# uber-research/deep-neuroevolution

Measured on NVIDIA H100. Metric: env-steps/sec across ES population (whole box), higher is better.
Workload: dtype f32

## Files before the change

### deep-neuroevolution_b200/csrc/gemv_bulk.cu

```cuda
#include <climits>
#include "common.cuh"
#include "forward.cuh"
#include "epilogue.cuh"
#include "wgmma.cuh"

using namespace wg;

int g_dne_gemv_bulk = 1;
int g_dne_gemv_ctas_per_sm = 2;
int g_dne_gemv_grid = 0;
int g_dne_gemv_stages = 5;

constexpr int GB_CONSUMERS = 256;
constexpr int GB_THREADS = GB_CONSUMERS + 32;
constexpr int GB_STAGES = 8;
constexpr int GB_STAGE_BYTES = 16384;
constexpr int GB_RPR = 4;
constexpr int GU_BLK = DNE_GEMV_BLOCK_ROWS;
constexpr int GU_VEC = 8;
constexpr int GU_VB = 4;
constexpr int GU_MIN_N = 64;
constexpr int GU_XS_LD_MAX = GU_BLK + 4096 / GU_MIN_N;
constexpr int GU_XS_FLOATS = GU_VEC * GU_XS_LD_MAX > (1024 / GU_MIN_N) * GU_VB * (GU_MIN_N + 4)
                                 ? GU_VEC * GU_XS_LD_MAX : (1024 / GU_MIN_N) * GU_VB * (GU_MIN_N + 4);
constexpr int GU_PLAN_BYTES_PER_GROUP = 8 + 5 * 4;

__device__ __forceinline__ int gu_cover(const int* pb0, const int* pb1, int n_groups, int b, int first, int cap, int* out,
                                        int lane) {
    int total = 0;
    for (int h0 = 0; h0 < n_groups; h0 += 32) {
        const int h = h0 + lane;
        const bool c = h < n_groups && pb0[h] <= b && b <= pb1[h];
        const unsigned m = __ballot_sync(0xffffffffu, c);
        const int ord = total + __popc(m & ((1u << lane) - 1u));
        if (c && ord >= first && ord < first + cap) out[ord - first] = h;
        total += __popc(m);
    }
    __syncwarp();
    return total;
}

template <int G>
__global__ void __launch_bounds__(GB_THREADS, 2)
gemv_union_kernel(SlotArgs sa, GemvSrc src, const float* __restrict__ X, int64_t x_slot_stride, int K, int N,
                  int n_pieces, int n_groups, int n_slots, float* __restrict__ part, int n_stages,
                  const float* __restrict__ tpart, int t_split) {
    constexpr int CAP = GU_VEC / G;
    extern __shared__ uint8_t smem_raw[];
    uint8_t* smem = (uint8_t*)(((uintptr_t)smem_raw + 127) & ~(uintptr_t)127);
    float* stage_base = reinterpret_cast<float*>(smem);
    int64_t* pE0 = reinterpret_cast<int64_t*>(smem + n_stages * GB_STAGE_BYTES);
    int* pb0 = reinterpret_cast<int*>(pE0 + n_groups);
    int* pb1 = pb0 + n_groups;
    int* psort = pb1 + n_groups;
    int* pstart = psort + n_groups;
    int* ppre = pstart + n_groups;
    __shared__ uint64_t full_bar[GB_STAGES], empty_bar[GB_STAGES];
    __shared__ __align__(16) float xs[GU_XS_FLOATS];
    __shared__ int cov_c[CAP], cov_p[CAP];
    __shared__ int rho_c[CAP];
    __shared__ int s_total, s_row0, s_nelem, s_items;

    const int tid = threadIdx.x, warp = tid >> 5, lane = tid & 31;
    const int NQ = N >> 2;
    const int RW = GB_CONSUMERS / NQ;
    const int RB = GB_RPR * RW;
    const int XS_LD = GU_BLK + RB;
    pdl_trigger();

    if (tid == 0) {
        for (int s = 0; s < n_stages; ++s) {
            mbar_init(&full_bar[s], 1);
            mbar_init(&empty_bar[s], GB_CONSUMERS / 32);
        }
        fence_mbar_init();
    }
    for (int g = tid; g < n_groups; g += GB_THREADS) {
        const int slot0 = g * G;
        bool any = false;
#pragma unroll
        for (int m = 0; m < G; ++m) any = any || (slot0 + m < n_slots && slot_active(sa, slot0 + m));
        const int64_t E0 = (src.idx64 ? src.idx64[slot0] : (src.idx32 ? (int64_t)src.idx32[slot0] * src.mul : 0)) + src.off;
        pE0[g] = E0;
        pb0[g] = any ? (int)(E0 / N / GU_BLK) : INT_MAX;
        pb1[g] = any ? (int)((E0 + (int64_t)K * N - 1) / N / GU_BLK) : -1;
    }
    __syncthreads();
    for (int g = tid; g < n_groups; g += GB_THREADS) {
        const int key = pb0[g];
        int r = 0;
        for (int h = 0; h < n_groups; ++h) {
            const int kh = pb0[h];
            r += (kh < key) || (kh == key && h < g);
        }
        psort[r] = g;
    }
    __syncthreads();
    if (warp == 0) {
        int carry_max = -1, carry_sum = 0;
        for (int i0 = 0; i0 < n_groups; i0 += 32) {
            const int i = i0 + lane;
            const int g = i < n_groups ? psort[i] : 0;
            const int b0 = i < n_groups ? pb0[g] : INT_MAX, b1 = i < n_groups ? pb1[g] : -1;
            int mx = b1;
#pragma unroll
            for (int d = 1; d < 32; d <<= 1) {
                const int o = __shfl_up_sync(0xffffffffu, mx, d);
                if (lane >= d) mx = max(mx, o);
            }
            int before = __shfl_up_sync(0xffffffffu, mx, 1);
            if (lane == 0) before = -1;
            before = max(before, carry_max);
            const int start = max(b0, before + 1);
            const int add = (b0 != INT_MAX && b1 >= start) ? b1 - start + 1 : 0;
            int sum = add;
#pragma unroll
            for (int d = 1; d < 32; d <<= 1) {
                const int o = __shfl_up_sync(0xffffffffu, sum, d);
                if (lane >= d) sum += o;
            }
            if (i < n_groups) { pstart[i] = start; ppre[i] = carry_sum + sum - add; }
            carry_sum += __shfl_sync(0xffffffffu, sum, 31);
            carry_max = max(carry_max, __shfl_sync(0xffffffffu, mx, 31));
        }
        if (lane == 0) s_items = carry_sum;
    }
    __syncthreads();
    const int n_items = s_items;
    auto item_block = [&](int q) {
        int lo = 0, hi = n_groups;
        while (lo < hi) {
            const int mid = (lo + hi) >> 1;
            if (ppre[mid] <= q) lo = mid + 1; else hi = mid;
        }
        return pstart[lo - 1] + (q - ppre[lo - 1]);
    };
    auto pass_range = [&](int b, const int* gl, int ng, int64_t& row0, int& n_elem) {
        int64_t r_first = INT64_MAX, e_last = 0;
        for (int i = 0; i < ng; ++i) {
            const int64_t E0 = pE0[gl[i]];
            r_first = min(r_first, E0 / N);
            e_last = max(e_last, (E0 + (int64_t)K * N + 3) & ~(int64_t)3);
        }
        const int64_t blk0 = (int64_t)b * GU_BLK;
        row0 = max(r_first, blk0);
        const int64_t e_end = min(e_last, (blk0 + GU_BLK) * N);
        n_elem = (int)(e_end - row0 * N);
    };

    if (warp == GB_CONSUMERS / 32) {
        uint32_t it = 0;
        for (int item = blockIdx.x; item < n_items; item += gridDim.x) {
            const int b = item_block(item);
            int total = CAP;
            for (int first = 0; first < total; first += CAP) {
                total = gu_cover(pb0, pb1, n_groups, b, first, CAP, cov_p, lane);
                int64_t row0;
                int n_elem;
                pass_range(b, cov_p, min(CAP, total - first), row0, n_elem);
                const float* gsrc = src.base + row0 * N;
                for (int e0 = 0; e0 < n_elem; e0 += RB * N, ++it) {
                    if (lane == 0) {
                        const int s = it % n_stages;
                        mbar_wait(&empty_bar[s], ((it / n_stages) & 1) ^ 1);
                        const uint32_t bytes = (uint32_t)min(RB * N, n_elem - e0) * 4;
                        mbar_arrive_expect_tx(&full_bar[s], bytes);
                        bulk_g2s(stage_base + (size_t)s * (GB_STAGE_BYTES / 4), gsrc + e0, bytes, &full_bar[s]);
                    }
                }
                __syncwarp();
            }
        }
        return;
    }

    pdl_wait();
    const int t = tid % NQ, rw = tid / NQ;
    const int red_ld = N + 4;
    float* red = xs;
    uint32_t it = 0;
    for (int item = blockIdx.x; item < n_items; item += gridDim.x) {
        const int b = item_block(item);
        int total = CAP;
        for (int first = 0; first < total; first += CAP) {
            if (warp == 0) {
                const int tot = gu_cover(pb0, pb1, n_groups, b, first, CAP, cov_c, lane);
                if (lane == 0) {
                    const int ng = min(CAP, tot - first);
                    int64_t row0;
                    int n_elem;
                    pass_range(b, cov_c, ng, row0, n_elem);
                    s_total = tot;
                    s_row0 = (int)(row0 - (int64_t)b * GU_BLK);
                    s_nelem = n_elem;
                    for (int i = 0; i < ng; ++i) rho_c[i] = (int)(pE0[cov_c[i]] % N);
                }
            }
            named_bar_sync(1, GB_CONSUMERS);
            total = s_total;
            const int ng = min(CAP, total - first), nv = ng * G;
            const int lrow0 = s_row0, n_elem = s_nelem;
            for (int i = tid; i < nv * XS_LD; i += GB_CONSUMERS) {
                const int v = i / XS_LD, L = i - v * XS_LD - 1;
                const int g = cov_c[v / G], slot = g * G + v % G;
                const int64_t k = (int64_t)b * GU_BLK + L - pE0[g] / N;
                xs[v * XS_LD + L + 1] = (k >= 0 && k < K && slot < n_slots) ? X[(int64_t)slot * x_slot_stride + k] : 0.0f;
            }
            named_bar_sync(1, GB_CONSUMERS);

            float acc[GU_VEC][4];
#pragma unroll
            for (int v = 0; v < GU_VEC; ++v)
#pragma unroll
                for (int c = 0; c < 4; ++c) acc[v][c] = 0.0f;

            for (int e0 = 0; e0 < n_elem; e0 += RB * N, ++it) {
                const int s = it % n_stages;
                const int stage_elems = min(RB * N, n_elem - e0);
                const int rl0 = rw * GB_RPR;
                const int xb0 = lrow0 + e0 / N + rl0;
                mbar_wait(&full_bar[s], (it / n_stages) & 1);
                const uint32_t rows_a = wg::smem_u32(stage_base) + s * GB_STAGE_BYTES + (rl0 * NQ + t) * 16;
                float4 w[GB_RPR];
#pragma unroll
                for (int j = 0; j < GB_RPR; ++j)
                    w[j] = ((rl0 + j) * N + 4 * t < stage_elems) ? wg::lds128(rows_a + j * NQ * 16) : make_float4(0.f, 0.f, 0.f, 0.f);
#pragma unroll
                for (int gi = 0; gi < CAP; ++gi) {
                    if (gi < ng) {
                        const int rho = rho_c[gi];
                        const bool p0 = 4 * t < rho, p1 = 4 * t + 1 < rho, p2 = 4 * t + 2 < rho, p3 = 4 * t + 3 < rho;
#pragma unroll
                        for (int m = 0; m < G; ++m) {
                            const int v = gi * G + m;
                            float xm[GB_RPR + 1];
#pragma unroll
                            for (int j = 0; j <= GB_RPR; ++j) xm[j] = xs[v * XS_LD + xb0 + j];
#pragma unroll
                            for (int j = 0; j < GB_RPR; ++j) {
                                acc[v][0] = fmaf(p0 ? xm[j] : xm[j + 1], w[j].x, acc[v][0]);
                                acc[v][1] = fmaf(p1 ? xm[j] : xm[j + 1], w[j].y, acc[v][1]);
                                acc[v][2] = fmaf(p2 ? xm[j] : xm[j + 1], w[j].z, acc[v][2]);
                                acc[v][3] = fmaf(p3 ? xm[j] : xm[j + 1], w[j].w, acc[v][3]);
                            }
                        }
                    }
                }
                __syncwarp();
                if (lane == 0) mbar_arrive(&empty_bar[s]);
            }
            for (int vb0 = 0; vb0 < nv; vb0 += GU_VB) {
                named_bar_sync(1, GB_CONSUMERS);
#pragma unroll
                for (int v = 0; v < GU_VEC; ++v) {
                    if (v >= vb0 && v < vb0 + GU_VB && v < nv) {
                        const int rho = rho_c[v / G];
                        float* row = red + (rw * GU_VB + (v - vb0)) * red_ld;
#pragma unroll
                        for (int c = 0; c < 4; ++c) {
                            const int n = 4 * t + c - rho;
                            row[n < 0 ? n + N : n] = acc[v][c];
                        }
                    }
                }
                named_bar_sync(1, GB_CONSUMERS);
                for (int i = tid; i < GU_VB * N; i += GB_CONSUMERS) {
                    const int vl = i / N, n = i - vl * N, v = vb0 + vl;
                    if (v >= nv) break;
                    const int g = cov_c[v / G], m = v % G, slot = g * G + m;
                    const int piece = b - pb0[g];
                    float sum = 0.0f;
                    for (int w2 = 0; w2 < RW; ++w2) sum += red[(w2 * GU_VB + vl) * red_ld + n];
                    if (tpart) {
                        float ts = 0.0f;
                        if (slot < n_slots)
                            for (int j = piece; j < t_split; j += n_pieces) ts += tpart[((int64_t)j * n_slots + slot) * N + n];
                        sum = fmaf(slot < n_slots ? sa.scale[slot] : 0.0f, sum, ts);
                    }
                    part[(((int64_t)g * n_pieces + piece) * G + m) * N + n] = sum;
                }
            }
            for (int gi = 0; gi < ng; ++gi) {
                const int g = cov_c[gi];
                if (pb1[g] != b) continue;
                for (int piece = b - pb0[g] + 1; piece < n_pieces; ++piece)
                    for (int i = tid; i < G * N; i += GB_CONSUMERS) {
                        const int m = i / N, n = i - m * N, slot = g * G + m;
                        float ts = 0.0f;
                        if (tpart && slot < n_slots)
                            for (int j = piece; j < t_split; j += n_pieces) ts += tpart[((int64_t)j * n_slots + slot) * N + n];
                        part[(((int64_t)g * n_pieces + piece) * G + m) * N + n] = ts;
                    }
            }
            named_bar_sync(1, GB_CONSUMERS);
        }
    }
}

int dne_gemv_pieces(int K) { return (K + 1 + GU_BLK - 1) / GU_BLK + 1; }

int dne_launch_gemv_union(const SlotArgs& sa, const GemvSrc& src, int G, const float* X, int64_t x_slot_stride, int K,
                          int N, int n_pieces, int n_slots, float* part, int sm_count, cudaStream_t st,
                          const float* fold_theta, int fold_n_split) {
    if (N % 4 != 0 || N < GU_MIN_N || N * 4 > GB_STAGE_BYTES || (GB_CONSUMERS % (N / 4)) != 0) return DNE_ERR_UNSUP;
    const int RW = GB_CONSUMERS / (N / 4);
    if (GB_RPR * RW * N * 4 != GB_STAGE_BYTES || n_pieces != dne_gemv_pieces(K) || (G != 1 && G != 2)) return DNE_ERR_UNSUP;
    const int n_groups = (n_slots + G - 1) / G;
    if (n_groups <= 0) return 0;
    const size_t static_smem = (size_t)GU_XS_FLOATS * 4 + 1024;
    const size_t plan = (size_t)n_groups * GU_PLAN_BYTES_PER_GROUP + 128;
    const size_t per_sm = 227 * 1024;
    int cps = g_dne_gemv_ctas_per_sm, n_stages = 0;
    for (; cps >= 1; --cps) {
        const size_t budget = per_sm / cps - 1024;
        n_stages = budget > static_smem + plan ? (int)((budget - static_smem - plan) / GB_STAGE_BYTES) : 0;
        if (n_stages > g_dne_gemv_stages) n_stages = g_dne_gemv_stages;
        if (n_stages >= 2) break;
    }
    if (cps < 1) return DNE_ERR_UNSUP;
    const size_t smem = (size_t)n_stages * GB_STAGE_BYTES + plan;
    int grid = cps * sm_count;
    if (g_dne_gemv_grid > 0 && grid > g_dne_gemv_grid) grid = g_dne_gemv_grid;
    int dev = 0;
    cudaGetDevice(&dev);
    static bool attr_done_dev[64][3] = {};
    bool* attr_done = attr_done_dev[dev < 64 ? dev : 63];
    auto launch = [&](auto kern) -> int {
        if (!attr_done[G]) {
            cudaFuncSetAttribute(kern, cudaFuncAttributePreferredSharedMemoryCarveout, cudaSharedmemCarveoutMaxShared);
            if (cudaFuncSetAttribute(kern, cudaFuncAttributeMaxDynamicSharedMemorySize, (int)(per_sm - static_smem - 1024)) != cudaSuccess)
                return DNE_ERR_CUDA;
            attr_done[G] = true;
        }
        if (dne_launch_chain(kern, dim3(grid), dim3(GB_THREADS), smem, st, true, sa, src, X, x_slot_stride, K, N, n_pieces,
                             n_groups, n_slots, part, n_stages, fold_theta, fold_theta ? fold_n_split : 0) != cudaSuccess)
            return DNE_ERR_CUDA;
        return 0;
    };
    return G == 2 ? launch(gemv_union_kernel<2>) : launch(gemv_union_kernel<1>);
}
```

Baseline: 345,300.

## Move x-vector staging to producer warp with double-buffered cp.async and mbarriers

The producer warp now computes pass metadata and loads the x-vector slices into a double-buffered shared buffer with cp.async zero-fill, signalling consumers through new mbarriers. This takes the cover computation, the x gather and two named barriers off the consumer critical path and lets the next pass's x load overlap the current pass's compute. It halves GU_VB so the reduction scratch fits inside one x buffer, which adds an extra reduction round for larger vector counts. Static shared memory grows because the x buffer is now doubled, which may cut the number of weight stages that fit.

```diff
diff --git a/deep-neuroevolution_b200/csrc/gemv_bulk.cu b/deep-neuroevolution_b200/csrc/gemv_bulk.cu
--- a/deep-neuroevolution_b200/csrc/gemv_bulk.cu
+++ b/deep-neuroevolution_b200/csrc/gemv_bulk.cu
@@ -18,12 +18,24 @@
 constexpr int GB_RPR = 4;
 constexpr int GU_BLK = DNE_GEMV_BLOCK_ROWS;
 constexpr int GU_VEC = 8;
-constexpr int GU_VB = 4;
+constexpr int GU_VB = 2;
 constexpr int GU_MIN_N = 64;
 constexpr int GU_XS_LD_MAX = GU_BLK + 4096 / GU_MIN_N;
-constexpr int GU_XS_FLOATS = GU_VEC * GU_XS_LD_MAX > (1024 / GU_MIN_N) * GU_VB * (GU_MIN_N + 4)
-                                 ? GU_VEC * GU_XS_LD_MAX : (1024 / GU_MIN_N) * GU_VB * (GU_MIN_N + 4);
+constexpr int GU_XS_BUF = GU_VEC * GU_XS_LD_MAX;
+static_assert((1024 / GU_MIN_N) * GU_VB * (GU_MIN_N + 4) <= GU_XS_BUF, "the reduction of every N fits an x buffer");
 constexpr int GU_PLAN_BYTES_PER_GROUP = 8 + 5 * 4;
+
+struct GuPass {
+    int b, total, ng, row0, n_elem;
+    int cov[GU_VEC], rho[GU_VEC];
+};
+
+__device__ __forceinline__ void cp_async4_zfill(float* dst, const float* src, bool ok) {
+    asm volatile("cp.async.ca.shared.global [%0], [%1], 4, %2;" ::"r"(smem_u32(dst)), "l"(src), "r"(ok ? 4 : 0) : "memory");
+}
+__device__ __forceinline__ void cp_async_mbar_arrive_noinc(uint64_t* bar) {
+    asm volatile("cp.async.mbarrier.arrive.noinc.shared::cta.b64 [%0];" ::"r"(smem_u32(bar)) : "memory");
+}
 
 __device__ __forceinline__ int gu_cover(const int* pb0, const int* pb1, int n_groups, int b, int first, int cap, int* out,
                                         int lane) {
@@ -38,6 +50,12 @@
     }
     __syncwarp();
     return total;
+}
+
+__device__ __forceinline__ void gu_pass_extent(int b, int64_t r_first, int64_t e_last, int N, int64_t& row0, int& n_elem) {
+    const int64_t blk0 = (int64_t)b * GU_BLK;
+    row0 = max(r_first, blk0);
+    n_elem = (int)(min(e_last, (blk0 + GU_BLK) * N) - row0 * N);
 }
 
 template <int G>
@@ -55,11 +73,11 @@
     int* psort = pb1 + n_groups;
     int* pstart = psort + n_groups;
     int* ppre = pstart + n_groups;
-    __shared__ uint64_t full_bar[GB_STAGES], empty_bar[GB_STAGES];
-    __shared__ __align__(16) float xs[GU_XS_FLOATS];
-    __shared__ int cov_c[CAP], cov_p[CAP];
-    __shared__ int rho_c[CAP];
-    __shared__ int s_total, s_row0, s_nelem, s_items;
+    __shared__ uint64_t full_bar[GB_STAGES], empty_bar[GB_STAGES], xs_full[2], xs_empty[2];
+    __shared__ __align__(16) float xs[2][GU_XS_BUF];
+    __shared__ GuPass pass[2];
+    __shared__ int cov_p[CAP];
+    __shared__ int s_items;
 
     const int tid = threadIdx.x, warp = tid >> 5, lane = tid & 31;
     const int NQ = N >> 2;
@@ -72,6 +90,10 @@
         for (int s = 0; s < n_stages; ++s) {
             mbar_init(&full_bar[s], 1);
             mbar_init(&empty_bar[s], GB_CONSUMERS / 32);
+        }
+        for (int s = 0; s < 2; ++s) {
+            mbar_init(&xs_full[s], 64);
+            mbar_init(&xs_empty[s], 1);
         }
         fence_mbar_init();
     }
@@ -135,39 +157,65 @@
         }
         return pstart[lo - 1] + (q - ppre[lo - 1]);
     };
-    auto pass_range = [&](int b, const int* gl, int ng, int64_t& row0, int& n_elem) {
-        int64_t r_first = INT64_MAX, e_last = 0;
-        for (int i = 0; i < ng; ++i) {
-            const int64_t E0 = pE0[gl[i]];
-            r_first = min(r_first, E0 / N);
-            e_last = max(e_last, (E0 + (int64_t)K * N + 3) & ~(int64_t)3);
-        }
-        const int64_t blk0 = (int64_t)b * GU_BLK;
-        row0 = max(r_first, blk0);
-        const int64_t e_end = min(e_last, (blk0 + GU_BLK) * N);
-        n_elem = (int)(e_end - row0 * N);
-    };
-
     if (warp == GB_CONSUMERS / 32) {
-        uint32_t it = 0;
+        uint32_t it = 0, p = 0;
+        auto issue = [&](const float* gsrc, int e0, int n_elem) {
+            if (lane == 0) {
+                const int s = it % n_stages;
+                mbar_wait(&empty_bar[s], ((it / n_stages) & 1) ^ 1);
+                const uint32_t bytes = (uint32_t)min(RB * N, n_elem - e0) * 4;
+                mbar_arrive_expect_tx(&full_bar[s], bytes);
+                bulk_g2s(stage_base + (size_t)s * (GB_STAGE_BYTES / 4), gsrc + e0, bytes, &full_bar[s]);
+            }
+            ++it;
+        };
         for (int item = blockIdx.x; item < n_items; item += gridDim.x) {
             const int b = item_block(item);
             int total = CAP;
-            for (int first = 0; first < total; first += CAP) {
+            for (int first = 0; first < total; first += CAP, ++p) {
                 total = gu_cover(pb0, pb1, n_groups, b, first, CAP, cov_p, lane);
-                int64_t row0;
+                const int ng = min(CAP, total - first);
+                int64_t r_first = INT64_MAX, e_last = 0, row0;
+                for (int j = 0; j < ng; ++j) {
+                    const int64_t E0 = pE0[cov_p[j]];
+                    r_first = min(r_first, E0 / N);
+                    e_last = max(e_last, (E0 + (int64_t)K * N + 3) & ~(int64_t)3);
+                }
                 int n_elem;
-                pass_range(b, cov_p, min(CAP, total - first), row0, n_elem);
+                gu_pass_extent(b, r_first, e_last, N, row0, n_elem);
                 const float* gsrc = src.base + row0 * N;
-                for (int e0 = 0; e0 < n_elem; e0 += RB * N, ++it) {
-                    if (lane == 0) {
-                        const int s = it % n_stages;
-                        mbar_wait(&empty_bar[s], ((it / n_stages) & 1) ^ 1);
-                        const uint32_t bytes = (uint32_t)min(RB * N, n_elem - e0) * 4;
-                        mbar_arrive_expect_tx(&full_bar[s], bytes);
-                        bulk_g2s(stage_base + (size_t)s * (GB_STAGE_BYTES / 4), gsrc + e0, bytes, &full_bar[s]);
-                    }
-                }
+                int e0 = 0;
+                if (p == 0) {
+                    for (; e0 < n_elem && e0 < n_stages * RB * N; e0 += RB * N) issue(gsrc, e0, n_elem);
+                    pdl_wait();
+                }
+                const int buf = p & 1;
+                mbar_wait(&xs_empty[buf], ((p >> 1) & 1) ^ 1);
+                if (lane < ng) {
+                    pass[buf].cov[lane] = cov_p[lane];
+                    pass[buf].rho[lane] = (int)(pE0[cov_p[lane]] % N);
+                }
+                if (lane == 0) {
+                    pass[buf].b = b;
+                    pass[buf].total = total;
+                    pass[buf].ng = ng;
+                    pass[buf].row0 = (int)(row0 - (int64_t)b * GU_BLK);
+                    pass[buf].n_elem = n_elem;
+                }
+                float* xb = xs[buf];
+                for (int v = 0; v < ng * G; ++v) {
+                    const int g = cov_p[v / G], slot = g * G + v % G;
+                    const int64_t k0 = (int64_t)b * GU_BLK - 1 - pE0[g] / N;
+                    const float* xrow = X + (int64_t)min(slot, n_slots - 1) * x_slot_stride;
+                    for (int j = lane; j < XS_LD; j += 32) {
+                        const int64_t k = k0 + j;
+                        const bool ok = slot < n_slots && k >= 0 && k < K;
+                        cp_async4_zfill(xb + v * XS_LD + j, ok ? xrow + k : X, ok);
+                    }
+                }
+                cp_async_mbar_arrive_noinc(&xs_full[buf]);
+                mbar_arrive(&xs_full[buf]);
+                for (; e0 < n_elem; e0 += RB * N) issue(gsrc, e0, n_elem);
                 __syncwarp();
             }
         }
@@ -177,36 +225,17 @@
     pdl_wait();
     const int t = tid % NQ, rw = tid / NQ;
     const int red_ld = N + 4;
-    float* red = xs;
-    uint32_t it = 0;
+    uint32_t it = 0, p = 0;
     for (int item = blockIdx.x; item < n_items; item += gridDim.x) {
-        const int b = item_block(item);
         int total = CAP;
-        for (int first = 0; first < total; first += CAP) {
-            if (warp == 0) {
-                const int tot = gu_cover(pb0, pb1, n_groups, b, first, CAP, cov_c, lane);
-                if (lane == 0) {
-                    const int ng = min(CAP, tot - first);
-                    int64_t row0;
-                    int n_elem;
-                    pass_range(b, cov_c, ng, row0, n_elem);
-                    s_total = tot;
-                    s_row0 = (int)(row0 - (int64_t)b * GU_BLK);
-                    s_nelem = n_elem;
-                    for (int i = 0; i < ng; ++i) rho_c[i] = (int)(pE0[cov_c[i]] % N);
-                }
-            }
-            named_bar_sync(1, GB_CONSUMERS);
-            total = s_total;
-            const int ng = min(CAP, total - first), nv = ng * G;
-            const int lrow0 = s_row0, n_elem = s_nelem;
-            for (int i = tid; i < nv * XS_LD; i += GB_CONSUMERS) {
-                const int v = i / XS_LD, L = i - v * XS_LD - 1;
-                const int g = cov_c[v / G], slot = g * G + v % G;
-                const int64_t k = (int64_t)b * GU_BLK + L - pE0[g] / N;
-                xs[v * XS_LD + L + 1] = (k >= 0 && k < K && slot < n_slots) ? X[(int64_t)slot * x_slot_stride + k] : 0.0f;
-            }
-            named_bar_sync(1, GB_CONSUMERS);
+        for (int first = 0; first < total; first += CAP, ++p) {
+            const int buf = p & 1;
+            mbar_wait(&xs_full[buf], (p >> 1) & 1);
+            const GuPass& ps = pass[buf];
+            total = ps.total;
+            const int ng = ps.ng, nv = ng * G;
+            const int lrow0 = ps.row0, n_elem = ps.n_elem;
+            const float* xb = xs[buf];
 
             float acc[GU_VEC][4];
 #pragma unroll
@@ -228,14 +257,14 @@
 #pragma unroll
                 for (int gi = 0; gi < CAP; ++gi) {
                     if (gi < ng) {
-                        const int rho = rho_c[gi];
+                        const int rho = ps.rho[gi];
                         const bool p0 = 4 * t < rho, p1 = 4 * t + 1 < rho, p2 = 4 * t + 2 < rho, p3 = 4 * t + 3 < rho;
 #pragma unroll
                         for (int m = 0; m < G; ++m) {
                             const int v = gi * G + m;
                             float xm[GB_RPR + 1];
 #pragma unroll
-                            for (int j = 0; j <= GB_RPR; ++j) xm[j] = xs[v * XS_LD + xb0 + j];
+                            for (int j = 0; j <= GB_RPR; ++j) xm[j] = xb[v * XS_LD + xb0 + j];
 #pragma unroll
                             for (int j = 0; j < GB_RPR; ++j) {
                                 acc[v][0] = fmaf(p0 ? xm[j] : xm[j + 1], w[j].x, acc[v][0]);
@@ -249,12 +278,13 @@
                 __syncwarp();
                 if (lane == 0) mbar_arrive(&empty_bar[s]);
             }
+            float* red = xs[buf];
             for (int vb0 = 0; vb0 < nv; vb0 += GU_VB) {
                 named_bar_sync(1, GB_CONSUMERS);
 #pragma unroll
                 for (int v = 0; v < GU_VEC; ++v) {
                     if (v >= vb0 && v < vb0 + GU_VB && v < nv) {
-                        const int rho = rho_c[v / G];
+                        const int rho = ps.rho[v / G];
                         float* row = red + (rw * GU_VB + (v - vb0)) * red_ld;
 #pragma unroll
                         for (int c = 0; c < 4; ++c) {
@@ -264,11 +294,11 @@
                     }
                 }
                 named_bar_sync(1, GB_CONSUMERS);
-                for (int i = tid; i < GU_VB * N; i += GB_CONSUMERS) {
-                    const int vl = i / N, n = i - vl * N, v = vb0 + vl;
+                for (int i2 = tid; i2 < GU_VB * N; i2 += GB_CONSUMERS) {
+                    const int vl = i2 / N, n = i2 - vl * N, v = vb0 + vl;
                     if (v >= nv) break;
-                    const int g = cov_c[v / G], m = v % G, slot = g * G + m;
-                    const int piece = b - pb0[g];
+                    const int g = ps.cov[v / G], m = v % G, slot = g * G + m;
+                    const int piece = ps.b - pb0[g];
                     float sum = 0.0f;
                     for (int w2 = 0; w2 < RW; ++w2) sum += red[(w2 * GU_VB + vl) * red_ld + n];
                     if (tpart) {
@@ -281,11 +311,11 @@
                 }
             }
             for (int gi = 0; gi < ng; ++gi) {
-                const int g = cov_c[gi];
-                if (pb1[g] != b) continue;
-                for (int piece = b - pb0[g] + 1; piece < n_pieces; ++piece)
-                    for (int i = tid; i < G * N; i += GB_CONSUMERS) {
-                        const int m = i / N, n = i - m * N, slot = g * G + m;
+                const int g = ps.cov[gi];
+                if (pb1[g] != ps.b) continue;
+                for (int piece = ps.b - pb0[g] + 1; piece < n_pieces; ++piece)
+                    for (int i2 = tid; i2 < G * N; i2 += GB_CONSUMERS) {
+                        const int m = i2 / N, n = i2 - m * N, slot = g * G + m;
                         float ts = 0.0f;
                         if (tpart && slot < n_slots)
                             for (int j = piece; j < t_split; j += n_pieces) ts += tpart[((int64_t)j * n_slots + slot) * N + n];
@@ -293,6 +323,7 @@
                     }
             }
             named_bar_sync(1, GB_CONSUMERS);
+            if (tid == 0) mbar_arrive(&xs_empty[buf]);
         }
     }
 }
@@ -307,7 +338,7 @@
     if (GB_RPR * RW * N * 4 != GB_STAGE_BYTES || n_pieces != dne_gemv_pieces(K) || (G != 1 && G != 2)) return DNE_ERR_UNSUP;
     const int n_groups = (n_slots + G - 1) / G;
     if (n_groups <= 0) return 0;
-    const size_t static_smem = (size_t)GU_XS_FLOATS * 4 + 1024;
+    const size_t static_smem = (size_t)2 * GU_XS_BUF * 4 + 1024;
     const size_t plan = (size_t)n_groups * GU_PLAN_BYTES_PER_GROUP + 128;
     const size_t per_sm = 227 * 1024;
     int cps = g_dne_gemv_ctas_per_sm, n_stages = 0;
```

Measured after the change: 350,900 (median of 6 runs). 1.6% higher.
